# AllenInstitute/distributed-vae

Hardware: AMD Instinct MI355X
Metric: cells/sec per train step (fwd+loss+bwd+opt) (higher is better)
Workload: dtype f32; 1 GPU; cpl_mixVAE A=2 arms, synthetic-10x-v1 50000 cells x 5000 genes per GPU, batch 5000/GPU, fp32, H=100 L=10 C=92 S=2, x_drop=0.5, Adam lr=1e-3; global_batch=5000, parallelism=dp1, noise=in-kernel Philox4x32-10

## Files before the change

distributed-vae_amd/_native.py:

```python
from __future__ import annotations

import ctypes as C
import os
from typing import Dict, Optional

import torch

HERE = os.path.dirname(os.path.abspath(__file__))
LIB_PATH = os.environ.get("MMVAE_LIB") or os.path.join(HERE, "libmmvae_hip.so")

ABI_VERSION = 5
N_PARAM_TENSORS = 28
N_BN = 6
MAX_ARMS = 8

PARAM_NAMES = [
    "fc1.weight", "fc1.bias", "fc2.weight", "fc2.bias", "fc3.weight", "fc3.bias", "fc4.weight", "fc4.bias",
    "fc5.weight", "fc5.bias", "fcc.weight", "fcc.bias", "fc_mu.weight", "fc_sigma.weight", "fc_mu.bias",
    "fc_sigma.bias", "fc6.weight", "fc6.bias", "fc7.weight", "fc7.bias", "fc8.weight", "fc8.bias",
    "fc9.weight", "fc9.bias", "fc10.weight", "fc10.bias", "fc11.weight", "fc11.bias",
]
BN_NAMES = ["batch_l1", "batch_l2", "batch_l3", "batch_l4", "batch_l5", "batch_s"]

WS_IDS = {name: i for i, name in enumerate([
# ... 54 lines not shown

def exec_from_env(engine: int = 0) -> Exec:
    ex = Exec()
    ex.tune[TUNE_ENGINE] = engine
    for w in range(6):
        v = os.environ.get(f"MMVAE_SPLIT{w}")
        if v:
            ex.split[w] = int(v)
    for name, (idx, conv) in TUNE_ENV.items():
        v = os.environ.get(name)
        if v:
            ex.tune[idx] = conv(v)
    return ex


class NativeError(RuntimeError):
    pass


PLAN_FIELDS = 23
PLAN_NAMES = ("kind", "fast", "big", "small_x3", "fc11", "gd10_slabs", "dw11_slabs", "chain_planes", "lat_half", "narrow",
              "presplit", "bwd_small_planes", "d10_planes", "dz1_in_apply", "dec_planes", "zero", "rowmap", "dz11_bf16",
              "dw11_side", "loss_on_side", "couple", "lat_fork_rides", "fc11_fork_rides")
CALL_KINDS = {"STEP": 0, "STEP_ROWS": 1, "FORWARD": 2, "BACKWARD": 3, "LOSS": 4, "CLASSIFY": 5, "REPLAY": 6, "DECODE": 7,
              "TRAVERSE": 8}
PLAN_ENUMS = {
    "big": ("GEMM_GENERAL", "GEMM_FP32", "GEMM_BF16", "GEMM_X3"),
    "fc11": ("FC11_GENERAL", "FC11_ZG", "FC11_ZT", "FC11_BF16", "FC11_X3", "FC11_OUT_BF16", "FC11_OUT_X3"),
    "zero": ("ZERO_NONE", "ZERO_MEMSET", "ZERO_XBITS", "ZERO_PRESPLIT"),
    "couple": ("COUPLE_INLINE", "COUPLE_SIDE", "COUPLE_IN_DEC"),
}


def debug_plan(dims: "Dims", hyper: "Hyper", ex: Optional["Exec"], kind: str, params_align: int = 16, x_align: int = 16,
               x_arm_stride: int = 0, has_x16: bool = False, fc11_grad: bool = True) -> Dict[str, object]:
    out = (C.c_int32 * PLAN_FIELDS)()
    check(lib().mmvae_debug_plan(C.byref(dims), C.byref(hyper), C.byref(ex) if ex is not None else None, CALL_KINDS[kind],
                                 int(params_align), int(x_align), int(x_arm_stride), int(bool(has_x16)), int(bool(fc11_grad)),
                                 C.byref(out)), "mmvae_debug_plan")
    plan = {}
    for name, v in zip(PLAN_NAMES, out):
        if name in PLAN_ENUMS:
            plan[name] = PLAN_ENUMS[name][v]
        elif name == "kind":
            plan[name] = next(k for k, i in CALL_KINDS.items() if i == v)
        elif name in ("gd10_slabs", "dw11_slabs"):
            plan[name] = int(v)
        else:
            plan[name] = bool(v)
    return plan


_lib = None


def lib():
    global _lib
    if _lib is not None:
        return _lib
    if not os.path.exists(LIB_PATH):
        raise NativeError(
            f"{LIB_PATH} not found: build the HIP extension first "
            "(python -c 'import __graft_entry__ as g; g.build()' or python distributed-vae_amd/build.py). "
            "There is no CPU fallback.")
    L = C.CDLL(LIB_PATH)
    vp, i64, f32, i32 = C.c_void_p, C.c_int64, C.c_float, C.c_int
    L.mmvae_abi_version.restype = C.c_int
    L.mmvae_last_error_string.restype = C.c_char_p
    L.mmvae_check_dims.argtypes = [C.POINTER(Dims)]
    L.mmvae_param_layout.argtypes = [C.POINTER(Dims), C.POINTER(ParamLayout)]
    ex = C.POINTER(Exec)
    L.mmvae_workspace_bytes.argtypes = [C.POINTER(Dims), ex]
    L.mmvae_workspace_bytes.restype = C.c_size_t
    L.mmvae_ws_offset.argtypes = [C.POINTER(Dims), ex, C.c_int]
    L.mmvae_ws_offset.restype = i64
    L.mmvae_splits.argtypes = [C.POINTER(Dims), ex, C.POINTER(C.c_int32 * 6)]
    L.mmvae_forward.argtypes = [C.POINTER(Dims), C.POINTER(Hyper), C.POINTER(Noise), vp, vp, vp, vp, i64, vp, i32,
                                vp, C.c_size_t, ex, vp]
    L.mmvae_loss.argtypes = [C.POINTER(Dims), C.POINTER(Hyper), vp, C.c_size_t, vp, ex, vp]
    L.mmvae_backward.argtypes = [C.POINTER(Dims), C.POINTER(Hyper), C.POINTER(Noise), vp, vp, i64, f32, vp,
                                 C.c_size_t, vp, ex, vp]
    L.mmvae_adam_step.argtypes = [i64, vp, vp, vp, vp, i64, f32, f32, f32, f32, f32, i32, vp]
    L.mmvae_train_step.argtypes = [C.POINTER(Dims), C.POINTER(Hyper), C.POINTER(Noise), vp, vp, vp, vp, i64, vp,
                                   C.c_size_t, vp, vp, i32, vp, vp, i64, f32, f32, f32, f32, f32, i32, ex, vp]
    L.mmvae_train_step_rows.argtypes = [C.POINTER(Dims), C.POINTER(Hyper), C.POINTER(Noise), vp, vp, vp, vp, vp, i64, i64, vp, vp,
                                        C.c_size_t, vp, vp, i32, vp, vp, i64, f32, f32, f32, f32, f32, i32, ex, vp]
    L.mmvae_train_step_rows.restype = C.c_int
    L.mmvae_to_bf16.argtypes = [vp, i64, i64, i32, vp, vp]
    L.mmvae_to_bf16.restype = C.c_int
    L.mmvae_debug_stage.argtypes = [C.POINTER(Dims), C.POINTER(Hyper), C.POINTER(Noise), i32, vp, vp, i64, vp,
                                    C.c_size_t, vp, ex, vp]
    L.mmvae_dump_noise.argtypes = [C.POINTER(Dims), C.POINTER(Hyper), C.POINTER(Noise), vp, vp, vp, vp, vp]
    L.mmvae_debug_plan.argtypes = [C.POINTER(Dims), C.POINTER(Hyper), ex, i32, i32, i32, i64, i32, i32,
                                   C.POINTER(C.c_int32 * PLAN_FIELDS)]
    L.mmvae_debug_plan.restype = C.c_int
    L.mmvae_eval_classify.argtypes = [C.POINTER(Dims), C.POINTER(Hyper), vp, vp, vp, i64, vp, C.c_size_t, vp, vp, ex,
                                      vp]
    L.mmvae_classify.argtypes = [vp, i64, i32, vp, vp]
    L.mmvae_confmat_accumulate.argtypes = [vp, i32, i64, i32, vp, vp]
    L.mmvae_consensus.argtypes = [vp, i32, i32, vp, vp, vp]
    L.mmvae_aug_packed_floats.argtypes = [C.POINTER(AugDims)]
    L.mmvae_aug_packed_floats.restype = C.c_size_t
    L.mmvae_aug_workspace_bytes.argtypes = [C.POINTER(AugDims), i32]
    L.mmvae_aug_workspace_bytes.restype = C.c_size_t
    L.mmvae_aug_pack.argtypes = [C.POINTER(AugDims), C.POINTER(AugTensors), vp, vp]
    L.mmvae_augment.argtypes = [C.POINTER(AugDims), vp, vp, i64, vp, vp, f32, vp, C.c_size_t, vp, vp, i32, ex, vp]
    L.mmvae_gather_rows.argtypes = [vp, i64, i64, vp, i64, i32, vp, vp]
    L.mmvae_tp_planes_bytes.argtypes = [i64, i32, i32]
    L.mmvae_tp_planes_bytes.restype = C.c_size_t
    L.mmvae_tp_planes.argtypes = [vp, i64, i64, i32, i32, vp, vp]
    L.mmvae_augment_rows.argtypes = [C.POINTER(AugDims), vp, vp, i64, i32, vp, vp, vp, f32, vp, C.c_size_t, vp, vp, i32, ex, vp]
    L.mmvae_decode_workspace_bytes.argtypes = [C.POINTER(Dims), ex]
    L.mmvae_decode_workspace_bytes.restype = C.c_size_t
    L.mmvae_decode.argtypes = [C.POINTER(Dims), C.POINTER(Hyper), vp, vp, i64, vp, i64, vp, vp, C.c_size_t, ex, vp]
    L.mmvae_decode.restype = C.c_int
    L.mmvae_state_changes_workspace_bytes.argtypes = [C.POINTER(Dims), i32, ex]
    L.mmvae_state_changes_workspace_bytes.restype = C.c_size_t
    L.mmvae_state_changes.argtypes = [C.POINTER(Dims), C.POINTER(Hyper), C.POINTER(Noise), vp, vp, vp, i32, i32, vp, vp,
# ... 330 lines not shown
```

distributed-vae_amd/csrc/api.hip:

```cpp
#include "common.hpp"
#include <stdarg.h>
#include <stdio.h>
#include <string.h>

namespace mmvae {

static thread_local char g_err[512] = "";
void set_error(const char* fmt, ...) {
    va_list ap;
    va_start(ap, fmt);
    vsnprintf(g_err, sizeof(g_err), fmt, ap);
    va_end(ap);
}

Splits default_splits(const mmvae_dims& d, const mmvae_exec* ex) {
    int g_split[6] = {0, 0, 0, 0, 0, 0};
    if (ex) for (int i = 0; i < 6; ++i) g_split[i] = ex->split[i] > 0 && ex->split[i] <= 64 ? ex->split[i] : 0;
    constexpr int CUS = 256;
    auto fit = [](int base_blocks, int slots, int cap) {
        const int base = base_blocks > 0 ? base_blocks : 1;
        auto eff = [&](int k) { const int n = base * k; return (double)n / (double)(((n + slots - 1) / slots) * slots); };
        int pick = 1;
        double best = 0.0;
        for (int k = 1; k <= cap; ++k) {
// ... 235 lines not shown
    else if (p.big == GEMM_X3 && fc11_grad && x3_fc11_fits(d) && slots) p.fc11 = FC11_X3;
    else if (p.big == GEMM_BF16) p.fc11 = FC11_BF16;
    else if (fc11_grad && d.H == 100 && (int64_t)cdiv(d.B, 256) * L.sp.ks_gd10 <= L.n11) p.fc11 = FC11_ZG;
    else p.fc11 = FC11_ZT;
    p.gd10_slabs = p.fast ? L.sp.ks_gd10 : L.sp.ns_fc11;
    p.dw11_slabs = p.fast ? L.sp.ks_dw11 : L.sp.ks_dw;
    p.chain_planes = p.fast && bf16_tiles && chain_planes_fit(d) && !c.tune(MMVAE_TUNE_CHAIN_FP32);
    p.lat_half = d.C <= 32 * LH_CPL && d.L <= 32 && 2 * d.S <= 32;
    p.narrow = h.gemm_bf16 == 1 && c.x16 != nullptr && bf16_tiles_fit(d) && (d.D & 7) == 0;
    p.presplit = fwd && p.fast && (x3 || p.chain_planes);
    p.bwd_small_planes = kind == CALL_BACKWARD && p.chain_planes;
    p.d10_planes = x3;
    p.dz1_in_apply = (x3 || p.narrow) && (d.H & 1) == 0;
    if (fwd && h.training) p.zero = p.presplit && dropout ? ZERO_PRESPLIT : p.fast && dropout ? ZERO_XBITS : ZERO_MEMSET;
    p.rowmap = kind == CALL_STEP_ROWS && p.zero == ZERO_PRESPLIT && slots && (p.fc11 == FC11_X3 || p.fc11 == FC11_BF16);
    p.dz11_bf16 = p.rowmap && c.x16 != nullptr && p.fc11 == FC11_BF16;
    p.dw11_side = (step || kind == CALL_BACKWARD) && p.fast && side;
    p.loss_on_side = step && p.fast && side;
    const int cs = c.tune(MMVAE_TUNE_COUPLE_SIDE);
    const bool role = p.loss_on_side && c.use_acc() && p.chain_planes && d.A >= 2 && d.A <= 5 && cs != 1 && (d.A >= 4 || cs == 3);
    p.couple = step && side ? (role ? COUPLE_IN_DEC : COUPLE_SIDE) : COUPLE_INLINE;
    p.lat_fork_rides = p.couple == COUPLE_SIDE && p.lat_half;
    p.fc11_fork_rides = p.loss_on_side && (p.fc11 == FC11_X3 || p.fc11 == FC11_BF16);
    if (kind == CALL_DECODE) {
        if (!p.fast) p.fc11 = FC11_GENERAL;
        else if (p.big == GEMM_X3 && x3_fc11_fits(d)) p.fc11 = FC11_OUT_X3;
        else if (p.big == GEMM_BF16) p.fc11 = FC11_OUT_BF16;
        else p.fc11 = FC11_ZT;
        p.d10_planes = p.fc11 == FC11_OUT_X3 || p.fc11 == FC11_OUT_BF16;
        p.dec_planes = p.d10_planes || p.chain_planes;
    }
}

static int fork_to_side(const Ctx& c, int ev) {
    if (hipEventRecord(c.ev(ev), c.stream) != hipSuccess || hipStreamWaitEvent(c.side(), c.ev(ev), 0) != hipSuccess) {
        set_error("stream fork failed");
        return MMVAE_E_LAUNCH;
    }
    return 0;
}
static int fork_wait_only(const Ctx& c, int ev) {
    if (hipStreamWaitEvent(c.side(), c.ev(ev), 0) != hipSuccess) { set_error("stream fork failed"); return MMVAE_E_LAUNCH; }
    return 0;
}
static int record_on_side(const Ctx& c, int ev) {
    if (hipEventRecord(c.ev(ev), c.side()) != hipSuccess) { set_error("event record failed"); return MMVAE_E_LAUNCH; }
// ... 424 lines not shown
        case 2: return fast ? launch_dw_big_fast(c, x, x_arm_stride, 3) : launch_dw_big(c, nz, x, x_arm_stride);
        case 9: return launch_make_xbits(c, nz);
        case 20: return launch_chain_fwd_enc(c, 3, params, nullptr, nullptr);
        case 21: return launch_chain_bwd_enc(c, 3, params);
        case 10: case 11: case 12: case 13: case 14:
            if (!fast) { set_error("stage %d needs the fast path", stage); return MMVAE_E_UNSUPPORTED; }
            if (stage == 10) return launch_fc11(c, params, x, x_arm_stride, nullptr, 1, 1);
            if (stage == 11) return launch_fc11(c, params, x, x_arm_stride, nullptr, 1, 2);
            if (stage == 12) return launch_dw_big_fast(c, x, x_arm_stride, 1);
            if (stage == 13) return launch_dw_big_fast(c, x, x_arm_stride, 2);
            return launch_fc1_fwd_fast(c, params, x, x_arm_stride);
        case 3: return launch_dw_small(c);
        case 4: return launch_chain_fwd_dec(c, params);
        case 5: return launch_chain_bwd_dec(c, params);
        case 6: return launch_lat_fwd(c, nz, params, nullptr, nullptr);
        case 7: return launch_lat_bwd(c, nz, params);
        case 8: if (!grads) { set_error("grads is null"); return MMVAE_E_BADARG; } return launch_reduce_grads(c, grads, 1.f, nullptr);
        default: set_error("unknown stage %d", stage); return MMVAE_E_BADARG;
    }
}

int mmvae_debug_plan(const mmvae_dims* d, const mmvae_hyper* h, const mmvae_exec* ex, int call_kind, int params_align,
                     int x_align, int64_t x_arm_stride, int has_x16, int fc11_grad, int32_t out[MMVAE_PLAN_FIELDS]) {
    if (int rc = check_dims(d)) return rc;
    if (!h || !out) { set_error("null hyper / out"); return MMVAE_E_BADARG; }
    if (int rc = check_gemm_engine(h->gemm_bf16)) return rc;
    static_assert(MMVAE_CALL_STEP == CALL_STEP && MMVAE_CALL_STEP_ROWS == CALL_STEP_ROWS && MMVAE_CALL_FORWARD == CALL_FORWARD &&
                  MMVAE_CALL_BACKWARD == CALL_BACKWARD && MMVAE_CALL_LOSS == CALL_LOSS && MMVAE_CALL_CLASSIFY == CALL_CLASSIFY &&
                  MMVAE_CALL_REPLAY == CALL_REPLAY && MMVAE_CALL_DECODE == CALL_DECODE && MMVAE_CALL_TRAVERSE == CALL_TRAVERSE,
                  "MMVAE_CALL_* (include/mmvae.h) are the values of CallKind");
    if (call_kind < CALL_STEP || call_kind > CALL_TRAVERSE) { set_error("unknown call kind %d", call_kind); return MMVAE_E_BADARG; }
    if (params_align < 0 || x_align < 0) { set_error("negative alignment"); return MMVAE_E_BADARG; }
    Ctx c{};
    c.d = *d;
    c.h = *h;
    if (call_kind == CALL_DECODE || call_kind == CALL_TRAVERSE || call_kind == CALL_CLASSIFY) c.h.training = 0;
    if (ex) c.ex = *ex; else memset(&c.ex, 0, sizeof(c.ex));
    c.lay = make_layout(*d, &c.ex);
    c.po = make_poff(*d);
    const uintptr_t base = 1u << 20;
    const float* params = reinterpret_cast<const float*>(base + (uintptr_t)(params_align & 15));
    const float* x = reinterpret_cast<const float*>(2 * base + (uintptr_t)(x_align & 15));
    if (has_x16 && call_kind == CALL_STEP_ROWS) c.x16 = reinterpret_cast<const unsigned short*>(3 * base);
    make_plan(c, (CallKind)call_kind, params, x, x_arm_stride, fc11_grad != 0);
    const Plan& p = c.plan;
    const int32_t v[] = {(int32_t)p.kind, p.fast, (int32_t)p.big, p.small_x3, (int32_t)p.fc11, p.gd10_slabs, p.dw11_slabs, p.chain_planes,
                         p.lat_half, p.narrow, p.presplit, p.bwd_small_planes, p.d10_planes, p.dz1_in_apply, p.dec_planes,
                         (int32_t)p.zero, p.rowmap, p.dz11_bf16, p.dw11_side, p.loss_on_side, (int32_t)p.couple, p.lat_fork_rides,
                         p.fc11_fork_rides};
    static_assert(sizeof(v) / sizeof(v[0]) == MMVAE_PLAN_FIELDS, "one value per field of Plan, in declaration order");
    for (int i = 0; i < MMVAE_PLAN_FIELDS; ++i) out[i] = v[i];
    return 0;
}

int mmvae_dump_noise(const mmvae_dims* d, const mmvae_hyper* h, const mmvae_noise* nz, uint8_t* x_mask,
                     float* u_gumbel, float* u_state, uint8_t* s_mask, void* stream) {
    if (int rc = check_dims(d)) return rc;
    if (!h || !nz) { set_error("null hyper / noise"); return MMVAE_E_BADARG; }
    return launch_dump_noise(*d, *h, nz, x_mask, u_gumbel, u_state, s_mask, reinterpret_cast<hipStream_t>(stream));
}

}
```

distributed-vae_amd/csrc/common.hpp:

```cpp
#pragma once
#include <hip/hip_runtime.h>
#include <hip/hip_ext.h>
#include <stdint.h>
#include "../../include/mmvae.h"
#include "tune.h"

namespace mmvae {

typedef float f32x16 __attribute__((ext_vector_type(16)));

constexpr int WAVE = 64;
constexpr int ROWS32 = 32;
constexpr int NP = 128;
constexpr int MAP_PAD = 256;
constexpr int DW11_LD = 132;
constexpr int SMALL_LD = 256;

__host__ __device__ inline int cdiv(int a, int b) { return (a + b - 1) / b; }
__host__ __device__ inline int64_t cdiv64(int64_t a, int64_t b) { return (a + b - 1) / b; }
__host__ __device__ inline int rup(int a, int b) { return cdiv(a, b) * b; }
__host__ __device__ inline int64_t imin64(int64_t a, int64_t b) { return a < b ? a : b; }

struct Splits {
    int ks_fc1;
// ... 563 lines not shown
                }
                const int left = D - 32 * w;
                if (left < 32) word &= (1u << left) - 1u;
                out[w] = word;
            }
        } else {
            const int w = tq, ncall = (int)(m >> 2), epc = 32 / ncall;
            uint32_t word = 0;
            for (int j = 0; j < ncall; ++j) {
                const u32x4 r = xmask_words(nz, arm, (uint32_t)row, (uint32_t)(w * ncall + j));
                for (int e = 0; e < epc; ++e) word |= xmask_field_keep(nz, r, (uint32_t)e) ? (1u << (j * epc + e)) : 0u;
            }
            const int left = D - 32 * w;
            if (left < 32) word &= (1u << left) - 1u;
            out[w] = word;
        }
    }
}
#endif

inline bool fast_dims(const mmvae_dims& d) { return (d.D & 3) == 0 && (d.H & 3) == 0; }
inline bool bf16_tiles_fit(const mmvae_dims& d) { return d.H <= 124; }
inline bool x3_fc11_fits(const mmvae_dims& d) { return d.H + 1 <= 112; }
inline bool chain_planes_fit(const mmvae_dims& d) { return d.C + d.S <= 128 && d.L <= 128; }
inline bool fc11_slots_fit(const Layout& L, int B) { return (int64_t)cdiv(B, 128) * L.sp.ks_gd10 <= L.n11; }

enum CallKind { CALL_STEP, CALL_STEP_ROWS, CALL_FORWARD, CALL_BACKWARD, CALL_LOSS, CALL_CLASSIFY, CALL_REPLAY ,
                CALL_DECODE , CALL_TRAVERSE  };
enum GemmFamily { GEMM_GENERAL, GEMM_FP32, GEMM_BF16, GEMM_X3 };
enum Fc11Family { FC11_GENERAL, FC11_ZG, FC11_ZT, FC11_BF16, FC11_X3, FC11_OUT_BF16, FC11_OUT_X3 };
enum FwdZero { ZERO_NONE, ZERO_MEMSET, ZERO_XBITS , ZERO_PRESPLIT  };
enum CouplePlace { COUPLE_INLINE, COUPLE_SIDE, COUPLE_IN_DEC };
struct Plan {
    CallKind kind;
    bool fast;
    GemmFamily big;
    bool small_x3;
    Fc11Family fc11;
    int gd10_slabs;
    int dw11_slabs;
    bool chain_planes;
    bool lat_half;
    bool narrow;
    bool presplit;
    bool bwd_small_planes;
    bool d10_planes;
    bool dz1_in_apply;
    bool dec_planes;
    FwdZero zero;
    bool rowmap;
    bool dz11_bf16;
    bool dw11_side;
    bool loss_on_side;
    CouplePlace couple;
    bool lat_fork_rides;
    bool fc11_fork_rides;
};

struct Ctx {
    mmvae_dims d;
    mmvae_hyper h;
    Layout lay;
    POff po;
    float* ws;
    hipStream_t stream;
    mmvae_exec ex;
    mmvae_exec* ex_out;
    hipStream_t side() const { return reinterpret_cast<hipStream_t>(ex.side_stream); }
    hipEvent_t ev(int i) const { return reinterpret_cast<hipEvent_t>(ex.ev[i]); }
    int tune(int i) const { return ex.tune[i]; }
    bool use_acc() const { return !ex.tune[MMVAE_TUNE_BN_PARTIALS]; }
    int64_t fwd_zero_floats() const { return acc_set_off(lay, d.A, ACC_BWD) - lay.fc11_part; }
    int64_t bwd_zero_floats() const { return lay.acc_end - acc_set_off(lay, d.A, ACC_BWD); }
    const int64_t* x_rows = nullptr;
    const unsigned short* x16 = nullptr;
    int64_t x_ld = 0, x_nrows = 0;
    Plan plan{};
    mutable hipEvent_t stop_ev = nullptr;
    mutable bool stop_used = false;
};
// ... 99 lines not shown
```

distributed-vae_amd/csrc/gemm_bf16.hip:

```cpp
#include "common.hpp"

namespace mmvae {

typedef __bf16 bf16x8 __attribute__((ext_vector_type(8)));
typedef __bf16 bf16x2 __attribute__((ext_vector_type(2)));
typedef unsigned int u32x4v __attribute__((ext_vector_type(4)));


constexpr int BT = 128;
constexpr int KT = 64;
constexpr int LDB = 36;
constexpr int LDK = 136;

template <int NP>
struct Eng {
    static constexpr int KT = NP == 1 ? 64 : 32;
    static constexpr int NQ = KT / 8;
    static constexpr int LDB = KT / 2 + 4;
    static constexpr int PLANE = BT * LDB;
    static constexpr int LDK = NP == 1 ? 136 : 160;
    static constexpr int NBUF = NP == 1 ? 2 : 1;
};

__device__ __forceinline__ unsigned pack_bf16(float a, float b) {
// ... 309 lines not shown
template <bool KMINOR>
__device__ __forceinline__ void plane_load(PlaneRegs& t, const PlaneDev& o, int r0, int k0, int j) {
    const int tid = threadIdx.x & 255, pl = j >> 1, id = tid + 256 * (j & 1);
    int off;
    if (!KMINOR) off = pl * o.plane + (r0 + (id >> 2)) * o.ld + k0 + 8 * (id & 3);
    else off = pl * o.plane + (k0 + (id >> 4)) * o.ld + r0 + 8 * (id & 15);
    t.v[j] = __builtin_bit_cast(u32x4v, __builtin_amdgcn_raw_buffer_load_b128(o.rs, off * 2, 0, 0));
}
template <bool KMINOR>
__device__ __forceinline__ void plane_store(unsigned* __restrict__ T, const PlaneRegs& t, int j) {
    const int tid = threadIdx.x & 255, pl = j >> 1, id = tid + 256 * (j & 1);
    int idx;
    if (!KMINOR) idx = pl * Eng<3>::PLANE + (id >> 2) * Eng<3>::LDB + 4 * (id & 3);
    else idx = pl * Eng<3>::PLANE + (((id >> 4) * Eng<3>::LDK + 8 * (id & 15)) >> 1);
    *reinterpret_cast<u32x4v*>(&T[idx]) = t.v[j];
}

struct SplitJob {
    const float* src; int64_t ld, src_arm;
    int R, C, Rp, Cp, ones_col;
    unsigned short* dst; int64_t dst_arm;
    const float* col_src; int64_t col_arm;
    int tr;
};
struct XbitsJob {
    NoiseDev nz; int A, B, D, wpr; uint32_t* bits; int blocks; float* zero_p; int zero_n4;
    const int64_t* rows; unsigned* map; int64_t rows_ld, n_rows;
};
struct SplitJobs { SplitJob j[24]; int first[25]; int n; XbitsJob xb; };
__global__ __launch_bounds__(256) void k_presplit(const SplitJobs js) {
    if (js.xb.zero_n4 > 0) grid_zero(js.xb.zero_p, js.xb.zero_n4);
    if (js.xb.rows && blockIdx.z == 0) {
        for (int i = blockIdx.x * 256 + threadIdx.x; i < js.xb.B + MAP_PAD; i += gridDim.x * 256) {
            const int64_t r = i < js.xb.B ? js.xb.rows[i] : 0;
            js.xb.map[i] = (unsigned)((r < 0 ? 0 : (r >= js.xb.n_rows ? js.xb.n_rows - 1 : r)) * js.xb.rows_ld);
        }
    }
    if ((int)blockIdx.x < js.xb.blocks) {
        make_xbits_range(js.xb.nz, js.xb.A, js.xb.B, js.xb.D, js.xb.wpr, js.xb.bits,
                         ((int64_t)blockIdx.z * js.xb.blocks + blockIdx.x) * 256 + threadIdx.x, (int64_t)gridDim.z * js.xb.blocks * 256);
        return;
    }
    const int bx0 = (int)blockIdx.x - js.xb.blocks;
    int ji = 0;
    while (ji + 1 < js.n && bx0 >= js.first[ji + 1]) ++ji;
    const SplitJob& J = js.j[ji];
    const int bx = bx0 - js.first[ji], nbx = js.first[ji + 1] - js.first[ji];
    const float* src = J.src + (int64_t)blockIdx.z * J.src_arm;
    const float* col = J.col_src ? J.col_src + (int64_t)blockIdx.z * J.col_arm : nullptr;
    unsigned short* dst = J.dst + (int64_t)blockIdx.z * J.dst_arm;
    const int c8n = J.Cp >> 3;
    const int64_t plane = (int64_t)J.Rp * J.Cp;
    const bool vec = (J.ld & 3) == 0 && (J.C & 3) == 0;
    const int n = J.Rp * c8n;
    for (int i = bx * 256 + threadIdx.x; i < n; i += nbx * 256) {
        const int r = i / c8n, c0 = (i - r * c8n) * 8;
        float v[8];
        if (J.tr) {
#pragma unroll
            for (int e = 0; e < 8; ++e) v[e] = (r < J.R && c0 + e < J.C) ? src[(int64_t)(c0 + e) * J.ld + r] : 0.f;
        } else if (r < J.R && vec && c0 + 8 <= J.C) {
            const float4 a = *reinterpret_cast<const float4*>(src + (int64_t)r * J.ld + c0);
            const float4 b = *reinterpret_cast<const float4*>(src + (int64_t)r * J.ld + c0 + 4);
            v[0] = a.x; v[1] = a.y; v[2] = a.z; v[3] = a.w; v[4] = b.x; v[5] = b.y; v[6] = b.z; v[7] = b.w;
        } else {
#pragma unroll
            for (int e = 0; e < 8; ++e) {
                const int c = c0 + e;
                v[e] = (r < J.R && c < J.C) ? src[(int64_t)r * J.ld + c] : ((r < J.R && c == J.ones_col) ? (col ? col[r] : 1.f) : 0.f);
            }
        }
        unsigned w[4][3];
#pragma unroll
        for (int e = 0; e < 4; ++e) split3(v[2 * e], v[2 * e + 1], w[e]);
#pragma unroll
        for (int pl = 0; pl < 3; ++pl)
            *reinterpret_cast<uint4*>(dst + pl * plane + (int64_t)r * J.Cp + c0) = make_uint4(w[0][pl], w[1][pl], w[2][pl], w[3][pl]);
    }
}

// ... 624 lines not shown
            const int h = 32 * nt + l31;
#pragma unroll
            for (int r = 0; r < 16; ++r) {
                const int row = c0 + 32 * wv + acc_row(r, lane);
                if (row < B && h < H) out[(int64_t)row * H + h] = gd[nt][r];
            }
        }
    }
    se = wave_sum(se);
    const float mf = wave_sum((float)mism);
    if (lane == 0) { red[wv * 2] = se; red[wv * 2 + 1] = mf; }
    __syncthreads();
    if (tid == 0) {
        float* p = g.fo.part + ((int64_t)arm * g.n11 + (int64_t)blockIdx.x * g.KS + blockIdx.y) * 2;
        p[0] = red[0] + red[2] + red[4] + red[6];
        p[1] = red[1] + red[3] + red[5] + red[7];
    }
}

constexpr int FW_ROW = 64;
constexpr int FW_PLANE = 64 * FW_ROW;
constexpr int FW_TILE = 3 * FW_PLANE;
__device__ __forceinline__ int fw_swz(int row) { return ((row & 3) << 2) | ((row >> 2) & 3); }
__global__ __launch_bounds__(256, 1) void k_x3_fc11g(const GemmArgs g_in) {
    const GemmArgs g = g_in;
    __shared__ __attribute__((aligned(16))) unsigned Wl[3 * FW_TILE];
    __shared__ float red[8];
    const int arm = blockIdx.z, tid = threadIdx.x, lane = tid & 63, wv = tid >> 6;
    const int l31 = lane & 31, hh = lane >> 5;
    const unsigned short* Wp = g.b.pl + (int64_t)arm * g.b.pl_arm;
    const unsigned short* Dp = g.a.pl + (int64_t)arm * g.a.pl_arm;
    const int64_t wplane = g.b.pl_plane, dplane = g.a.pl_plane;
    const int B = g.fo.B, D = g.fo.D, H = g.K;
    const int c0 = blockIdx.x * 128;
    const int tiles = cdiv(D, 64);
    const int t0 = (int)(((int64_t)blockIdx.y * tiles) / g.KS), t1 = (int)(((int64_t)(blockIdx.y + 1) * tiles) / g.KS);
    const int cell = c0 + 32 * wv + l31;
    const float* xa = g.fo.x + (int64_t)arm * g.fo_x_arm;
    float* dza = g.fo.dz + (int64_t)arm * g.fo_arm;
    const __amdgpu_buffer_rsrc_t rx = __builtin_amdgcn_make_buffer_rsrc(const_cast<float*>(xa), 0, (int)((g.fo.xmap ? g.fo.x_nrec : (int64_t)B * D) * 4), 0x00020000);
    const __amdgpu_buffer_rsrc_t rz = __builtin_amdgcn_make_buffer_rsrc(dza, 0, (int)((int64_t)B * D * 4), 0x00020000);
    const int rowoff = g.fo.xmap ? (int)g.fo.xmap[min(cell, B - 1)] : min(cell, B - 1) * D;
    const bool cell_ok = cell < B;
    int dzoff = min(cell, B - 1) * D * 4;
    asm volatile("" : "+v"(dzoff));
    int dlim = cell_ok ? D : 0;
// ... 150 lines not shown
            if (s < 5) chunk(s);
        }
        asm volatile("" : "+s"(mism));
        if (dma_tile >= 0) dma(dma_tile);
#pragma unroll
        for (int r = 0; r < 4; ++r) {
            __builtin_amdgcn_sched_barrier(0);
            if (r + 1 < 4) d_frags(Wt16, r + 1);
            if (r >= 2) {
                const unsigned* W2 = w_rows(p + 2 < npieces ? p + 2 : p);
                z_frags(W2, r - 2);
            }
            if (r == 0) { chunk(5); chunk(6); }
            if (r == 1) chunk(7);
            const int c = r >> 1;
            bf16x8 af[3];
#pragma unroll
            for (int pl = 0; pl < 3; ++pl) {
                u32x4v u;
                u[0] = au[c][pl][0]; u[1] = au[c][pl][1]; u[2] = au[c][pl][2]; u[3] = au[c][pl][3];
                af[pl] = __builtin_bit_cast(bf16x8, u);
            }
            const int n0 = 2 * (r & 1);
#pragma unroll
            for (int j = 0; j < 2; ++j) gd[n0 + j] = __builtin_amdgcn_mfma_f32_32x32x16_bf16(af[2], wq[r & 1][j][0], gd[n0 + j], 0, 0, 0);
#pragma unroll
            for (int j = 0; j < 2; ++j) gd[n0 + j] = __builtin_amdgcn_mfma_f32_32x32x16_bf16(af[0], wq[r & 1][j][2], gd[n0 + j], 0, 0, 0);
#pragma unroll
            for (int j = 0; j < 2; ++j) gd[n0 + j] = __builtin_amdgcn_mfma_f32_32x32x16_bf16(af[1], wq[r & 1][j][1], gd[n0 + j], 0, 0, 0);
#pragma unroll
            for (int j = 0; j < 2; ++j) gd[n0 + j] = __builtin_amdgcn_mfma_f32_32x32x16_bf16(af[1], wq[r & 1][j][0], gd[n0 + j], 0, 0, 0);
#pragma unroll
            for (int j = 0; j < 2; ++j) gd[n0 + j] = __builtin_amdgcn_mfma_f32_32x32x16_bf16(af[0], wq[r & 1][j][1], gd[n0 + j], 0, 0, 0);
#pragma unroll
            for (int j = 0; j < 2; ++j) gd[n0 + j] = __builtin_amdgcn_mfma_f32_32x32x16_bf16(af[0], wq[r & 1][j][0], gd[n0 + j], 0, 0, 0);
        }
        __builtin_amdgcn_sched_barrier(0);
    };
    for (int t = t0; t < t1; ++t) {
        const int p = 2 * (t - t0);
        piece(p, acc_a, xa_, xb_, (t > t0 && t + 2 < t1) ? t + 2 : -1);
        piece(p + 1, acc_a, xb_, xa_, -1);
        __builtin_amdgcn_s_waitcnt(0x0F74);
        __syncthreads();
    }
    {
        float* out = g.so.out + (int64_t)blockIdx.y * g.so.ks_stride + (int64_t)arm * g.so.arm_stride;
#pragma unroll
        for (int nt = 0; nt < 4; ++nt) {
            const int h = 32 * nt + l31;
#pragma unroll
            for (int r = 0; r < 16; ++r) {
                const int row = c0 + 32 * wv + acc_row(r, lane);
                if (row < B && h < H) out[(int64_t)row * H + h] = gd[nt][r];
            }
        }
    }
    const float se = wave_sum((seq[0] + seq[1]) + (seq[2] + seq[3]));
    if (lane == 0) { red[wv * 2] = se; red[wv * 2 + 1] = (float)mism; }
    __syncthreads();
    if (tid == 0) {
        float* pp = g.fo.part + ((int64_t)arm * g.n11 + (int64_t)blockIdx.x * g.KS + blockIdx.y) * 2;
        pp[0] = (red[0] + red[2]) + (red[4] + red[6]);
        pp[1] = (red[1] + red[3]) + (red[5] + red[7]);
    }
    if (blockIdx.x == 0 && blockIdx.y == 0)
        for (int i = (int)gridDim.x * g.KS * 2 + tid; i < 2 * g.n11; i += 256) g.fo.part[(int64_t)arm * g.n11 * 2 + i] = 0.f;
}

struct Fc11OutArgs {
// ... 141 lines not shown
static Operand kmajor(const float* p, int64_t ld, int rows, int K) { return Operand{p, ld, rows, K, 0, nullptr, 0, -1, nullptr, 0, 0, 0, nullptr, 0, 0, 0}; }
static Operand kminor(const float* p, int64_t ld, int rows, int K) { return Operand{p, ld, rows, K, 1, nullptr, 0, -1, nullptr, 0, 0, 0, nullptr, 0, 0, 0}; }

static inline int rup_i(int a, int b) { return cdiv(a, b) * b; }
enum { PL_W1 = 0, PL_W11 = 1, PL_D10 = 2, PL_DZ1 = 3 };
struct PlaneGeom { int R, C, Rp, Cp, ones_col; int64_t ws_off; };
static PlaneGeom plane_geom(const Ctx& c, int kind) {
    const mmvae_dims& d = c.d;
    switch (kind) {
        case PL_W1:  return PlaneGeom{d.H, d.D, 128, rup_i(d.D, 32), -1, c.lay.pl_w1};
        case PL_W11: return PlaneGeom{d.D, d.H, rup_i(d.D, 128), 128, d.H, c.lay.pl_w11};
        case PL_D10: return PlaneGeom{d.B, d.H, rup_i(d.B, 256), 128, d.H, c.lay.pl_d10};
        default:     return PlaneGeom{d.B, d.H, rup_i(d.B, 256), 128, -1, c.lay.pl_dz1};
    }
}
static void use_planes(const Ctx& c, Operand& o, int kind) {
    const PlaneGeom g = plane_geom(c, kind);
    o.pl = reinterpret_cast<const unsigned short*>(c.ws + g.ws_off);
    o.pl_plane = (int64_t)g.Rp * g.Cp; o.pl_arm = 3 * o.pl_plane; o.pl_ld = g.Cp;
}
static SplitJob plane_job(const Ctx& c, int kind, const float* src, int64_t ld, int64_t src_arm, const float* col_src = nullptr, int64_t col_arm = 0) {
    const PlaneGeom g = plane_geom(c, kind);
    return SplitJob{src, ld, src_arm, g.R, g.C, g.Rp, g.Cp, g.ones_col, reinterpret_cast<unsigned short*>(c.ws + g.ws_off),
                    3 * (int64_t)g.Rp * g.Cp, col_src, col_arm};
}
static int launch_presplit(hipStream_t s, int A, const SplitJob* jobs, int n, const XbitsJob* xb = nullptr) {
    SplitJobs js{};
    if (xb) js.xb = *xb;
    js.n = n;
    for (int i = 0; i < n; ++i) {
        js.j[i] = jobs[i];
        js.first[i + 1] = js.first[i] + (int)imin64(1024, cdiv64((int64_t)jobs[i].Rp * (jobs[i].Cp / 8), 256));
    }
    hipLaunchKernelGGL(k_presplit, dim3(js.xb.blocks + js.first[n], 1, A), dim3(256), 0, s, js);
    HIP_LAUNCH_CHECK("k_presplit");
    return 0;
}

int launch_x3_planes(const Ctx& c, const float* params, bool head, const mmvae_noise* nz) {
    const Plan& p = c.plan;
    XbitsJob xb{};
    const bool xbits = head && p.zero == ZERO_PRESPLIT;
    if (xbits) {
        const mmvae_dims& dd = c.d;
        xb.nz = make_noise_dev(nz, c.h);
        xb.A = dd.A; xb.B = dd.B; xb.D = dd.D; xb.wpr = cdiv(dd.D, 32);
        xb.bits = reinterpret_cast<uint32_t*>(c.ws + c.lay.xbits);
// ... 113 lines not shown

int launch_fc11_bf16(const Ctx& c, const float* params, const float* x, int64_t xs, float* x_rec, int need_grad, int which) {
    const mmvae_dims& d = c.d;
    const Layout& L = c.lay;
    const int NS = L.sp.ks_gd10;
    const bool fused = need_grad && !x_rec;
    if (c.plan.fc11 == FC11_X3) {
        if (!(which & 1)) return 0;
        GemmArgs g{};
        g.a = kmajor(c.ws + L.Dk[4], d.H, d.B, d.H);
        g.b = kmajor(params + c.po.o[26], d.H, d.D, d.H);
        use_planes(c, g.b, PL_W11);
        use_planes(c, g.a, PL_D10);
        g.M = d.B; g.N = d.D; g.K = d.H; g.KS = NS; g.A = d.A; g.n11 = L.n11;
        g.fo = Fc11Out{params + c.po.o[27], x, c.ws + L.DZ11, nullptr, c.ws + L.fc11_part,
                       (float)(d.A > 1 ? d.A - 1 : 1) / (float)d.B, d.B, d.D, nullptr, 0};
        if (c.plan.rowmap) {
            g.fo.xmap = reinterpret_cast<const unsigned*>(c.ws + L.rowmap);
            g.fo.x_nrec = c.x_nrows * c.x_ld;
        }
        g.fo_arm = (int64_t)d.B * d.D;
        g.fo_x_arm = xs;
        g.so = SlabOut{c.ws + L.GD10_slab, (int64_t)d.A * d.B * d.H, (int64_t)d.B * d.H, d.H, d.B, d.H};
        launch_k(c, k_x3_fc11g, dim3(cdiv(d.B, 128), NS, d.A), dim3(256), 0, g);
        HIP_LAUNCH_CHECK("k_x3_fc11g");
        return 0;
    }
    if (which & 1) {
        hipError_t e = c.plan.zero != ZERO_NONE ? hipSuccess : hipMemsetAsync(c.ws + L.fc11_part, 0, sizeof(float) * 2 * (size_t)d.A * L.n11, c.stream);
        if (e != hipSuccess) { set_error("memset: %s", hipGetErrorString(e)); return MMVAE_E_LAUNCH; }
        if (!fc11_slots_fit(L, d.B)) { set_error("fc11 bf16: loss partial slots"); return MMVAE_E_LAUNCH; }
        GemmArgs g{};
        g.a = kmajor(c.ws + L.Dk[4], d.H, d.B, d.H);
        g.a_arm = (int64_t)d.B * d.H;
        g.b = kmajor(params + c.po.o[26], d.H, d.D, d.H);
        g.b_arm = c.po.per_arm;
        g.bias_arm = c.po.per_arm;
        g.M = d.B; g.N = d.D; g.K = d.H; g.KS = NS; g.A = d.A; g.n11 = L.n11;
        g.fo = Fc11Out{params + c.po.o[27], x, c.ws + L.DZ11, x_rec, c.ws + L.fc11_part,
                       (float)(d.A > 1 ? d.A - 1 : 1) / (float)d.B, d.B, d.D, nullptr, 0};
        if (c.plan.rowmap) {
            g.fo.xmap = reinterpret_cast<const unsigned*>(c.ws + L.rowmap);
            g.fo.x_nrec = c.x_nrows * c.x_ld;
        }
        g.fo_arm = (int64_t)d.B * d.D;
        g.fo_x_arm = xs;
        if (fused) {
// ... 103 lines not shown
```

include/mmvae.h:

```cpp
#ifndef MMVAE_H
#define MMVAE_H

#include <stddef.h>
#include <stdint.h>

#ifdef __cplusplus
extern "C" {
#endif

#define MMVAE_OK 0
#define MMVAE_E_BADARG (-1)
#define MMVAE_E_UNSUPPORTED (-2)
#define MMVAE_E_LAUNCH (-3)
#define MMVAE_E_WORKSPACE (-4)

#define MMVAE_MAX_ARMS 8
#define MMVAE_N_PARAM_TENSORS 28
#define MMVAE_N_BN 6

typedef struct mmvae_dims {
    int32_t A, B, D, H, L, C, S;
} mmvae_dims;

typedef struct mmvae_hyper {
// ... 177 lines not shown
                        mmvae_exec *ex, void *stream);

int mmvae_dump_noise(const mmvae_dims *d, const mmvae_hyper *h, const mmvae_noise *nz,
                     uint8_t *x_mask, float *u_gumbel, float *u_state, uint8_t *s_mask,
                     void *stream);

int mmvae_debug_stage(const mmvae_dims *d, const mmvae_hyper *h, const mmvae_noise *nz, int stage,
                      const float *params, const float *x, int64_t x_arm_stride, void *ws,
                      size_t ws_bytes, float *grads, mmvae_exec *ex, void *stream);

#define MMVAE_PLAN_FIELDS 23
#define MMVAE_CALL_STEP 0
#define MMVAE_CALL_STEP_ROWS 1
#define MMVAE_CALL_FORWARD 2
#define MMVAE_CALL_BACKWARD 3
#define MMVAE_CALL_LOSS 4
#define MMVAE_CALL_CLASSIFY 5
#define MMVAE_CALL_REPLAY 6
#define MMVAE_CALL_DECODE 7
#define MMVAE_CALL_TRAVERSE 8
int mmvae_debug_plan(const mmvae_dims *d, const mmvae_hyper *h, const mmvae_exec *ex, int call_kind,
                     int params_align, int x_align, int64_t x_arm_stride, int has_x16, int fc11_grad,
                     int32_t out[MMVAE_PLAN_FIELDS]);

#ifdef __cplusplus
}
#endif
#endif
```

Measured before the change: 7.531 million cells/s.

## Pack fc11 weight tail columns into spare plane slots to skip MFMA tiles

With H=100, the fc11 gradient kernel's fourth 32-column N tile holds only four live columns. The change packs those tail columns of the W11 bf16 split planes, grouped by split level, into the padding columns beyond column 112. This lets the last tile skip several of the split-precision MFMA products, which a single extra MFMA and a lane-permute reduction in the epilogue then recombine. It cuts MFMA work in k_x3_fc11g at the cost of a more complex plane layout, an epilogue shuffle, and a template-specialised kernel.

```diff
diff --git a/distributed-vae_amd/_native.py b/distributed-vae_amd/_native.py
--- a/distributed-vae_amd/_native.py
+++ b/distributed-vae_amd/_native.py
@@ -100,6 +100,9 @@
 PLAN_NAMES = ("kind", "fast", "big", "small_x3", "fc11", "gd10_slabs", "dw11_slabs", "chain_planes", "lat_half", "narrow",
               "presplit", "bwd_small_planes", "d10_planes", "dz1_in_apply", "dec_planes", "zero", "rowmap", "dz11_bf16",
               "dw11_side", "loss_on_side", "couple", "lat_fork_rides", "fc11_fork_rides")
+PLAN_FIELDS_EXT = 24
+PLAN_NAMES_EXT = PLAN_NAMES + ("tail_pack",)
+TAIL_PACK = ("unpacked", "packed")
 CALL_KINDS = {"STEP": 0, "STEP_ROWS": 1, "FORWARD": 2, "BACKWARD": 3, "LOSS": 4, "CLASSIFY": 5, "REPLAY": 6, "DECODE": 7,
               "TRAVERSE": 8}
 PLAN_ENUMS = {
@@ -126,6 +129,17 @@
             plan[name] = int(v)
         else:
             plan[name] = bool(v)
+    return plan
+
+
+def debug_plan_ext(dims: "Dims", hyper: "Hyper", ex: Optional["Exec"], kind: str, **kw) -> Dict[str, object]:
+    plan = debug_plan(dims, hyper, ex, kind, **kw)
+    out = (C.c_int32 * PLAN_FIELDS_EXT)()
+    check(lib().mmvae_debug_plan_ext(C.byref(dims), C.byref(hyper), C.byref(ex) if ex is not None else None, CALL_KINDS[kind],
+                                     int(kw.get("params_align", 16)), int(kw.get("x_align", 16)), int(kw.get("x_arm_stride", 0)),
+                                     int(bool(kw.get("has_x16", False))), int(bool(kw.get("fc11_grad", True))), C.byref(out)),
+          "mmvae_debug_plan_ext")
+    plan["tail_pack"] = TAIL_PACK[out[PLAN_FIELDS]]
     return plan
 
 
@@ -172,6 +186,10 @@
     L.mmvae_debug_plan.argtypes = [C.POINTER(Dims), C.POINTER(Hyper), ex, i32, i32, i32, i64, i32, i32,
                                    C.POINTER(C.c_int32 * PLAN_FIELDS)]
     L.mmvae_debug_plan.restype = C.c_int
+    if hasattr(L, "mmvae_debug_plan_ext"):
+        L.mmvae_debug_plan_ext.argtypes = [C.POINTER(Dims), C.POINTER(Hyper), ex, i32, i32, i32, i64, i32, i32,
+                                           C.POINTER(C.c_int32 * PLAN_FIELDS_EXT)]
+        L.mmvae_debug_plan_ext.restype = C.c_int
     L.mmvae_eval_classify.argtypes = [C.POINTER(Dims), C.POINTER(Hyper), vp, vp, vp, i64, vp, C.c_size_t, vp, vp, ex,
                                       vp]
     L.mmvae_classify.argtypes = [vp, i64, i32, vp, vp]
diff --git a/distributed-vae_amd/csrc/api.hip b/distributed-vae_amd/csrc/api.hip
--- a/distributed-vae_amd/csrc/api.hip
+++ b/distributed-vae_amd/csrc/api.hip
@@ -281,6 +281,7 @@
     p.couple = step && side ? (role ? COUPLE_IN_DEC : COUPLE_SIDE) : COUPLE_INLINE;
     p.lat_fork_rides = p.couple == COUPLE_SIDE && p.lat_half;
     p.fc11_fork_rides = p.loss_on_side && (p.fc11 == FC11_X3 || p.fc11 == FC11_BF16);
+    p.tail_pack = (p.big == GEMM_X3 && x3_fc11_fits(d) && x3_tail_pack_t(d.H) > 0) ? TAIL_W11 : TAIL_NONE;
     if (kind == CALL_DECODE) {
         if (!p.fast) p.fc11 = FC11_GENERAL;
         else if (p.big == GEMM_X3 && x3_fc11_fits(d)) p.fc11 = FC11_OUT_X3;
@@ -751,6 +752,14 @@
 
 int mmvae_debug_plan(const mmvae_dims* d, const mmvae_hyper* h, const mmvae_exec* ex, int call_kind, int params_align,
                      int x_align, int64_t x_arm_stride, int has_x16, int fc11_grad, int32_t out[MMVAE_PLAN_FIELDS]) {
+    int32_t all[MMVAE_PLAN_FIELDS_EXT];
+    if (int rc = mmvae_debug_plan_ext(d, h, ex, call_kind, params_align, x_align, x_arm_stride, has_x16, fc11_grad, out ? all : nullptr)) return rc;
+    for (int i = 0; i < MMVAE_PLAN_FIELDS; ++i) out[i] = all[i];
+    return 0;
+}
+
+int mmvae_debug_plan_ext(const mmvae_dims* d, const mmvae_hyper* h, const mmvae_exec* ex, int call_kind, int params_align,
+                         int x_align, int64_t x_arm_stride, int has_x16, int fc11_grad, int32_t out[MMVAE_PLAN_FIELDS_EXT]) {
     if (int rc = check_dims(d)) return rc;
     if (!h || !out) { set_error("null hyper / out"); return MMVAE_E_BADARG; }
     if (int rc = check_gemm_engine(h->gemm_bf16)) return rc;
@@ -776,9 +785,9 @@
     const int32_t v[] = {(int32_t)p.kind, p.fast, (int32_t)p.big, p.small_x3, (int32_t)p.fc11, p.gd10_slabs, p.dw11_slabs, p.chain_planes,
                          p.lat_half, p.narrow, p.presplit, p.bwd_small_planes, p.d10_planes, p.dz1_in_apply, p.dec_planes,
                          (int32_t)p.zero, p.rowmap, p.dz11_bf16, p.dw11_side, p.loss_on_side, (int32_t)p.couple, p.lat_fork_rides,
-                         p.fc11_fork_rides};
-    static_assert(sizeof(v) / sizeof(v[0]) == MMVAE_PLAN_FIELDS, "one value per field of Plan, in declaration order");
-    for (int i = 0; i < MMVAE_PLAN_FIELDS; ++i) out[i] = v[i];
+                         p.fc11_fork_rides, p.tail_pack};
+    static_assert(sizeof(v) / sizeof(v[0]) == MMVAE_PLAN_FIELDS_EXT, "one value per field of Plan, in declaration order");
+    for (int i = 0; i < MMVAE_PLAN_FIELDS_EXT; ++i) out[i] = v[i];
     return 0;
 }
 
diff --git a/distributed-vae_amd/csrc/common.hpp b/distributed-vae_amd/csrc/common.hpp
--- a/distributed-vae_amd/csrc/common.hpp
+++ b/distributed-vae_amd/csrc/common.hpp
@@ -609,6 +609,11 @@
 inline bool fast_dims(const mmvae_dims& d) { return (d.D & 3) == 0 && (d.H & 3) == 0; }
 inline bool bf16_tiles_fit(const mmvae_dims& d) { return d.H <= 124; }
 inline bool x3_fc11_fits(const mmvae_dims& d) { return d.H + 1 <= 112; }
+constexpr int X3_PACK_COL = 112;
+inline int x3_tail_pack_t(int n) {
+    const int t = n & 31;
+    return (n > 96 && n <= 128 && t > 0 && t <= 8 && n <= X3_PACK_COL && X3_PACK_COL + 2 * t <= 128) ? t : 0;
+}
 inline bool chain_planes_fit(const mmvae_dims& d) { return d.C + d.S <= 128 && d.L <= 128; }
 inline bool fc11_slots_fit(const Layout& L, int B) { return (int64_t)cdiv(B, 128) * L.sp.ks_gd10 <= L.n11; }
 
@@ -642,7 +647,9 @@
     CouplePlace couple;
     bool lat_fork_rides;
     bool fc11_fork_rides;
+    int tail_pack;
 };
+enum TailPack { TAIL_NONE = 0, TAIL_W11 = 1  };
 
 struct Ctx {
     mmvae_dims d;
diff --git a/distributed-vae_amd/csrc/gemm_bf16.hip b/distributed-vae_amd/csrc/gemm_bf16.hip
--- a/distributed-vae_amd/csrc/gemm_bf16.hip
+++ b/distributed-vae_amd/csrc/gemm_bf16.hip
@@ -355,6 +355,7 @@
     unsigned short* dst; int64_t dst_arm;
     const float* col_src; int64_t col_arm;
     int tr;
+    int pack_t;
 };
 struct XbitsJob {
     NoiseDev nz; int A, B, D, wpr; uint32_t* bits; int blocks; float* zero_p; int zero_n4;
@@ -389,6 +390,25 @@
     for (int i = bx * 256 + threadIdx.x; i < n; i += nbx * 256) {
         const int r = i / c8n, c0 = (i - r * c8n) * 8;
         float v[8];
+        if (J.pack_t > 0 && c0 >= X3_PACK_COL) {
+            const int t = J.pack_t;
+            unsigned o[3][8];
+#pragma unroll
+            for (int e = 0; e < 8; ++e) {
+                const int g = c0 + e - X3_PACK_COL, grp = g < t ? 1 : (g < 2 * t ? 2 : 0);
+                const float sv = (grp && r < J.R) ? src[(int64_t)r * J.ld + (J.C - grp * t + g)] : 0.f;
+                unsigned w3[3];
+                split3(sv, 0.f, w3);
+                o[0][e] = grp == 1 ? (w3[1] & 0xFFFFu) : (w3[2] & 0xFFFFu);
+                o[1][e] = grp == 1 ? (w3[0] & 0xFFFFu) : 0u;
+                o[2][e] = o[1][e];
+            }
+#pragma unroll
+            for (int pl = 0; pl < 3; ++pl)
+                *reinterpret_cast<uint4*>(dst + pl * plane + (int64_t)r * J.Cp + c0) =
+                    make_uint4(o[pl][0] | (o[pl][1] << 16), o[pl][2] | (o[pl][3] << 16), o[pl][4] | (o[pl][5] << 16), o[pl][6] | (o[pl][7] << 16));
+            continue;
+        }
         if (J.tr) {
 #pragma unroll
             for (int e = 0; e < 8; ++e) v[e] = (r < J.R && c0 + e < J.C) ? src[(int64_t)(c0 + e) * J.ld + r] : 0.f;
@@ -1059,6 +1079,7 @@
 constexpr int FW_PLANE = 64 * FW_ROW;
 constexpr int FW_TILE = 3 * FW_PLANE;
 __device__ __forceinline__ int fw_swz(int row) { return ((row & 3) << 2) | ((row >> 2) & 3); }
+template <bool PACK>
 __global__ __launch_bounds__(256, 1) void k_x3_fc11g(const GemmArgs g_in) {
     const GemmArgs g = g_in;
     __shared__ __attribute__((aligned(16))) unsigned Wl[3 * FW_TILE];
@@ -1255,16 +1276,18 @@
                 af[pl] = __builtin_bit_cast(bf16x8, u);
             }
             const int n0 = 2 * (r & 1);
-#pragma unroll
-            for (int j = 0; j < 2; ++j) gd[n0 + j] = __builtin_amdgcn_mfma_f32_32x32x16_bf16(af[2], wq[r & 1][j][0], gd[n0 + j], 0, 0, 0);
-#pragma unroll
-            for (int j = 0; j < 2; ++j) gd[n0 + j] = __builtin_amdgcn_mfma_f32_32x32x16_bf16(af[0], wq[r & 1][j][2], gd[n0 + j], 0, 0, 0);
+            const int nj = (PACK && (r & 1)) ? 1 : 2;
+#pragma unroll
+            for (int j = 0; j < nj; ++j) gd[n0 + j] = __builtin_amdgcn_mfma_f32_32x32x16_bf16(af[2], wq[r & 1][j][0], gd[n0 + j], 0, 0, 0);
+            if (nj == 1) gd[3] = __builtin_amdgcn_mfma_f32_32x32x16_bf16(af[2], wq[1][1][2], gd[3], 0, 0, 0);
+#pragma unroll
+            for (int j = 0; j < nj; ++j) gd[n0 + j] = __builtin_amdgcn_mfma_f32_32x32x16_bf16(af[0], wq[r & 1][j][2], gd[n0 + j], 0, 0, 0);
 #pragma unroll
             for (int j = 0; j < 2; ++j) gd[n0 + j] = __builtin_amdgcn_mfma_f32_32x32x16_bf16(af[1], wq[r & 1][j][1], gd[n0 + j], 0, 0, 0);
 #pragma unroll
-            for (int j = 0; j < 2; ++j) gd[n0 + j] = __builtin_amdgcn_mfma_f32_32x32x16_bf16(af[1], wq[r & 1][j][0], gd[n0 + j], 0, 0, 0);
-#pragma unroll
-            for (int j = 0; j < 2; ++j) gd[n0 + j] = __builtin_amdgcn_mfma_f32_32x32x16_bf16(af[0], wq[r & 1][j][1], gd[n0 + j], 0, 0, 0);
+            for (int j = 0; j < nj; ++j) gd[n0 + j] = __builtin_amdgcn_mfma_f32_32x32x16_bf16(af[1], wq[r & 1][j][0], gd[n0 + j], 0, 0, 0);
+#pragma unroll
+            for (int j = 0; j < nj; ++j) gd[n0 + j] = __builtin_amdgcn_mfma_f32_32x32x16_bf16(af[0], wq[r & 1][j][1], gd[n0 + j], 0, 0, 0);
 #pragma unroll
             for (int j = 0; j < 2; ++j) gd[n0 + j] = __builtin_amdgcn_mfma_f32_32x32x16_bf16(af[0], wq[r & 1][j][0], gd[n0 + j], 0, 0, 0);
         }
@@ -1279,6 +1302,16 @@
     }
     {
         float* out = g.so.out + (int64_t)blockIdx.y * g.so.ks_stride + (int64_t)arm * g.so.arm_stride;
+        if (PACK) {
+            const int t = H - 96;
+            const int s1 = 4 * ((lane + 16) & 63), s2 = 4 * ((lane + 16 + t) & 63);
+#pragma unroll
+            for (int r = 0; r < 16; ++r) {
+                const int v = __float_as_int(gd[3][r]);
+                const float g1 = __int_as_float(__builtin_amdgcn_ds_bpermute(s1, v)), g2 = __int_as_float(__builtin_amdgcn_ds_bpermute(s2, v));
+                gd[3][r] = (g2 + g1) + gd[3][r];
+            }
+        }
 #pragma unroll
         for (int nt = 0; nt < 4; ++nt) {
             const int h = 32 * nt + l31;
@@ -1466,7 +1499,8 @@
 static SplitJob plane_job(const Ctx& c, int kind, const float* src, int64_t ld, int64_t src_arm, const float* col_src = nullptr, int64_t col_arm = 0) {
     const PlaneGeom g = plane_geom(c, kind);
     return SplitJob{src, ld, src_arm, g.R, g.C, g.Rp, g.Cp, g.ones_col, reinterpret_cast<unsigned short*>(c.ws + g.ws_off),
-                    3 * (int64_t)g.Rp * g.Cp, col_src, col_arm};
+                    3 * (int64_t)g.Rp * g.Cp, col_src, col_arm, 0,
+                    kind == PL_W11 && (c.plan.tail_pack & TAIL_W11) ? x3_tail_pack_t(g.C) : 0};
 }
 static int launch_presplit(hipStream_t s, int A, const SplitJob* jobs, int n, const XbitsJob* xb = nullptr) {
     SplitJobs js{};
@@ -1626,7 +1660,8 @@
         g.fo_arm = (int64_t)d.B * d.D;
         g.fo_x_arm = xs;
         g.so = SlabOut{c.ws + L.GD10_slab, (int64_t)d.A * d.B * d.H, (int64_t)d.B * d.H, d.H, d.B, d.H};
-        launch_k(c, k_x3_fc11g, dim3(cdiv(d.B, 128), NS, d.A), dim3(256), 0, g);
+        if (c.plan.tail_pack & TAIL_W11) launch_k(c, k_x3_fc11g<true>, dim3(cdiv(d.B, 128), NS, d.A), dim3(256), 0, g);
+        else launch_k(c, k_x3_fc11g<false>, dim3(cdiv(d.B, 128), NS, d.A), dim3(256), 0, g);
         HIP_LAUNCH_CHECK("k_x3_fc11g");
         return 0;
     }
diff --git a/include/mmvae.h b/include/mmvae.h
--- a/include/mmvae.h
+++ b/include/mmvae.h
@@ -223,6 +223,10 @@
 int mmvae_debug_plan(const mmvae_dims *d, const mmvae_hyper *h, const mmvae_exec *ex, int call_kind,
                      int params_align, int x_align, int64_t x_arm_stride, int has_x16, int fc11_grad,
                      int32_t out[MMVAE_PLAN_FIELDS]);
+#define MMVAE_PLAN_FIELDS_EXT 24
+int mmvae_debug_plan_ext(const mmvae_dims *d, const mmvae_hyper *h, const mmvae_exec *ex, int call_kind,
+                         int params_align, int x_align, int64_t x_arm_stride, int has_x16, int fc11_grad,
+                         int32_t out[MMVAE_PLAN_FIELDS_EXT]);
 
 #ifdef __cplusplus
 }
```

Result: no change. 7.523 million cells/s (-0.1%).
